# zzuiekongning/MGDT-YOLO

Hardware: AMD Instinct MI355X
Metric: images/sec @640x640 bs=32 per GPU, detection forward + NMS (whole job: 1 GPU(s)) (higher is better)
Workload: dtype bf16; 1 GPU; mspa_c2f_gd_yolov8-n (MSPA-C2f + GD neck + Detect, nc=80) 640x640 inference, batch 32/GPU: forward + decode + NMS(conf 0.25, iou 0.7), hipGraph replay, 4 batches in flight (one captured graph per resident batch, replayed round-robin on 4 streams); global_batch=32, parallelism=replicas x1 (batch-sharded, no data-path collective), rccl_ranks=1, input=bfloat16 NCHW images, 8 different batches resident in HBM (600 MiB) cycled, detections_last_step=9600, weights=seeded random init (no checkpoints offline), batches_in_flight=4

## Files before the change

### mgdt_yolo_amd/csrc/inject_fused.hip

```cpp
#include "conv_igemm_kernel.h"

struct InjArgs {
  const char* x; int xsn, xsh, xsw; uint32_t x_bytes;
  const char* ga; const char* gf; int gsn, gsh, gsw;
  char* y; int ysn, ysh, ysw; uint32_t y_bytes;
  const char* wpk; const float* bias;
  int N, H, W, Cin, Cout, Hg, Wg, PH, PW, tiles_x, tiles_y;
  FastDiv fd_tx, fd_ty;
  float ry, rx;
};

constexpr int INJ_TH = 4, INJ_TW = 16, INJ_THREADS = 256, INJ_CPAD = 8;

__device__ __host__ inline void inj_lerp_r(int o, float scale, int isz, int& i0, int& i1, float& l1) {
#pragma clang fp contract(off)
  float src = scale * ((float)o + 0.5f) - 0.5f;
  if (src < 0.f) src = 0.f;
  i0 = (int)src;
  if (i0 > isz - 1) i0 = isz - 1;
  i1 = i0 + (i0 < isz - 1 ? 1 : 0);
  l1 = src - (float)i0;
}
__device__ __host__ inline void inj_lerp(int o, int isz, int osz, int& i0, int& i1, float& l1) {
#pragma clang fp contract(off)
  inj_lerp_r(o, (float)isz / (float)osz, isz, i0, i1, l1);
}

typedef __attribute__((ext_vector_type(2))) float inj_f32x2;
typedef __attribute__((ext_vector_type(2))) __bf16 inj_bf16x2;
typedef __attribute__((ext_vector_type(4))) unsigned int u32x4;
__device__ __forceinline__ uint32_t inj_pk_bf16(float lo, float hi) {
  return __builtin_bit_cast(uint32_t, __builtin_convertvector(inj_f32x2{lo, hi}, inj_bf16x2));
}
__device__ __forceinline__ float inj_bf16_lo(uint32_t w) { return __uint_as_float(w << 16); }
__device__ __forceinline__ float inj_bf16_hi(uint32_t w) { return __uint_as_float(w & 0xffff0000u); }

struct InjGeo { int n, ty, tx, py0, px0, ph, pw; uint32_t pwm; };
__device__ __forceinline__ uint32_t inj_pw_magic(int pw) {
  uint32_t m = (uint32_t)(65536.f * __builtin_amdgcn_rcpf((float)pw));
  m -= (m * (uint32_t)pw > 65536u);
  m += ((m + 1) * (uint32_t)pw <= 65536u);
  return m + 1;
}
template <int TH>
__device__ __forceinline__ InjGeo inj_geom(const InjArgs& a, int patch) {
  InjGeo q;
  const uint32_t row = fdiv((uint32_t)patch, a.fd_tx);
  q.tx = patch - (int)row * a.tiles_x;
  q.n = (int)fdiv(row, a.fd_ty);
  q.ty = (int)row - q.n * a.tiles_y;
  int py1, px1, t0, t1; float tl;
  inj_lerp_r(q.ty * TH, a.ry, a.Hg, q.py0, t1, tl);
  inj_lerp_r(min(q.ty * TH + TH - 1, a.H - 1), a.ry, a.Hg, t0, py1, tl);
  inj_lerp_r(q.tx * INJ_TW, a.rx, a.Wg, q.px0, t1, tl);
  inj_lerp_r(min(q.tx * INJ_TW + INJ_TW - 1, a.W - 1), a.rx, a.Wg, t0, px1, tl);
  q.ph = py1 - q.py0 + 1; q.pw = px1 - q.px0 + 1;
  q.pwm = inj_pw_magic(q.pw);
  return q;
}

template <typename T, int KC, int NB>
__global__ __launch_bounds__(INJ_THREADS) void conv1x1_inject_kernel(const InjArgs a) {
  typedef typename Piece<T>::frag frag;
  constexpr int SZ = (int)sizeof(T);
  constexpr int CS = NB * 16 + INJ_CPAD;
  extern __shared__ __attribute__((aligned(16))) char smem[];
  char* wl = smem;
  T* sg = (T*)(smem + (size_t)KC * NB * 1024);
  T* sf = sg + (size_t)a.PH * a.PW * CS;
  const int tid = threadIdx.x, lane = tid & 63;
  const int wave = __builtin_amdgcn_readfirstlane(tid >> 6);
  const int r = lane & 15, g = lane >> 4;
  for (int i = tid; i < KC * NB * 64; i += INJ_THREADS) ((uint4*)wl)[i] = ((const uint4*)a.wpk)[i];
  const __amdgpu_buffer_rsrc_t xrs = __builtin_amdgcn_make_buffer_rsrc((void*)a.x, 0, a.x_bytes, 0x00020000);
  const __amdgpu_buffer_rsrc_t yrs = __builtin_amdgcn_make_buffer_rsrc((void*)a.y, 0, a.y_bytes, 0x00020000);
  const char* const wlane = wl + lane * 16;
  const int npatch = a.N * a.tiles_x * a.tiles_y;
#pragma unroll 1
  for (int patch = blockIdx.x; patch < npatch; patch += gridDim.x) {
  const InjGeo q = inj_geom<INJ_TH>(a, patch);
  const int n = q.n, ty = q.ty, tx = q.tx, py0 = q.py0, px0 = q.px0, ph = q.ph, pw = q.pw;
  const int oy = ty * INJ_TH + wave, ox = tx * INJ_TW + r;
  const bool pv = oy < a.H && ox < a.W;

  const int xo = pv ? n * a.xsn + oy * a.xsh + ox * a.xsw : MGDT_OOB;
  frag P[KC];
#pragma unroll
  for (int kc = 0; kc < KC; ++kc) {
    const int cb = (kc * 4 + g) * 16;
    P[kc] = __builtin_bit_cast(frag, __builtin_amdgcn_raw_buffer_load_b128(xrs, (cb < a.Cin * SZ) ? (uint32_t)(xo + cb) : (uint32_t)MGDT_OOB, 0, 0));
  }
  __syncthreads();
  {
    constexpr int VPP = NB * 16 / 8;
    const int nvec = ph * pw * VPP;
    for (int i = tid; i < nvec; i += INJ_THREADS) {
      const int v = i % VPP, p = i / VPP;
      const int sy = (int)(((uint32_t)p * q.pwm) >> 16), sx = p - sy * pw;
      const long go = (long)n * a.gsn + (long)(py0 + sy) * a.gsh + (long)(px0 + sx) * a.gsw + v * 16;
      const uint4 va = *(const uint4*)(a.ga + go), vf = *(const uint4*)(a.gf + go);
      *(uint4*)((char*)sg + ((size_t)p * CS + v * 8) * SZ) = va;
      *(uint4*)((char*)sf + ((size_t)p * CS + v * 8) * SZ) = vf;
    }
  }
  __syncthreads();

  f32x4 acc[NB];
#pragma unroll
  for (int nb = 0; nb < NB; ++nb) acc[nb] = *(const f32x4*)(a.bias + nb * 16 + 4 * g);
#pragma unroll
  for (int kc = 0; kc < KC; ++kc)
#pragma unroll
    for (int nb = 0; nb < NB; ++nb) acc[nb] = mma(*(const frag*)(wlane + (kc * NB + nb) * 1024), P[kc], acc[nb]);

  int y0, y1, x0, x1; float wy1, wx1;
  inj_lerp_r(min(oy, a.H - 1), a.ry, a.Hg, y0, y1, wy1);
  inj_lerp_r(min(ox, a.W - 1), a.rx, a.Wg, x0, x1, wx1);
  const int o00 = ((y0 - py0) * pw + (x0 - px0)) * CS + 4 * g, o01 = ((y0 - py0) * pw + (x1 - px0)) * CS + 4 * g;
  const int o10 = ((y1 - py0) * pw + (x0 - px0)) * CS + 4 * g, o11 = ((y1 - py0) * pw + (x1 - px0)) * CS + 4 * g;
  const int yo = pv ? n * a.ysn + oy * a.ysh + ox * a.ysw : MGDT_OOB;
  auto ld = [&](const T* base, int off) __attribute__((always_inline)) {
    const bf16x4 v = *(const bf16x4*)(base + off);
    return f32x4{(float)v[0], (float)v[1], (float)v[2], (float)v[3]};
  };
  auto hs = [](f32x4 v) __attribute__((always_inline)) {
    f32x4 o;
#pragma unroll
    for (int j = 0; j < 4; ++j) o[j] = fminf(fmaxf(fmaf(v[j], 1.f / 6.f, 0.5f), 0.f), 1.f);
    return o;
  };
#pragma unroll
  for (int nb = 0; nb < NB; ++nb) {
    const int c = nb * 16;
    const f32x4 sig = (hs(ld(sg, o00 + c)) * (1.f - wx1) + hs(ld(sg, o01 + c)) * wx1) * (1.f - wy1) +
                      (hs(ld(sg, o10 + c)) * (1.f - wx1) + hs(ld(sg, o11 + c)) * wx1) * wy1;
    const f32x4 feat = (ld(sf, o00 + c) * (1.f - wx1) + ld(sf, o01 + c) * wx1) * (1.f - wy1) +
                       (ld(sf, o10 + c) * (1.f - wx1) + ld(sf, o11 + c) * wx1) * wy1;
    f32x4 loc;
#pragma unroll
    for (int j = 0; j < 4; ++j) loc[j] = (float)(T)acc[nb][j];
    bstore4<T>(yrs, (uint32_t)yo + (uint32_t)((c + 4 * g) * SZ), loc * sig + feat);
  }
  }
}

struct InjConvArgs {
  InjArgs a;
  const char* gx; int gxsn, gxsh, gxsw; uint32_t gx_bytes;
  const char* wg; const float* bias_g;
  const char* w2; const float* bias2;
  char* y2; int y2sn, y2sh, y2sw; uint32_t y2_bytes;
  int C2, act2;
};

template <int KC, int NB, int NB2, int TH, bool GCONV>
__global__ __launch_bounds__(64 * TH) void conv1x1_inject_conv_kernel(const InjConvArgs A) {
  typedef bf16 T;
  typedef bf16x8 frag;
  const InjArgs& a = A.a;
  constexpr int SZ = 2, THREADS = 64 * TH;
  constexpr int CS = NB * 16 + INJ_CPAD;
  constexpr int KC2 = NB / 2;
  extern __shared__ __attribute__((aligned(16))) char smem[];
  char* wl = smem;
  char* w2l = smem + (size_t)KC * NB * 1024;
  T* sg = (T*)(w2l + (size_t)KC2 * NB2 * 1024);
  T* sf = sg + (size_t)a.PH * a.PW * CS;
  char* hgT = (char*)sg;
  char* gfT = hgT + (size_t)NB * 2 * 1024;

  const int tid = threadIdx.x, lane = tid & 63;
  const int wave = __builtin_amdgcn_readfirstlane(tid >> 6);
  const int r = lane & 15, g = lane >> 4;
  {
    constexpr int W1 = KC * NB * 64, W2 = KC2 * NB2 * 64, N1 = (W1 + THREADS - 1) / THREADS, N2 = (W2 + THREADS - 1) / THREADS;
    uint4 t1[N1], t2[N2];
#pragma unroll
    for (int u = 0; u < N1; ++u) t1[u] = ((const uint4*)a.wpk)[min(tid + u * THREADS, W1 - 1)];
#pragma unroll
    for (int u = 0; u < N2; ++u) t2[u] = ((const uint4*)A.w2)[min(tid + u * THREADS, W2 - 1)];
#pragma unroll
    for (int u = 0; u < N1; ++u) if (tid + u * THREADS < W1) ((uint4*)wl)[tid + u * THREADS] = t1[u];
#pragma unroll
    for (int u = 0; u < N2; ++u) if (tid + u * THREADS < W2) ((uint4*)w2l)[tid + u * THREADS] = t2[u];
  }
  if (GCONV) {
    for (int i = tid; i < NB * 2 * 2 * 64; i += THREADS) ((uint4*)hgT)[i] = make_uint4(0u, 0u, 0u, 0u);
  }
  const __amdgpu_buffer_rsrc_t xrs = __builtin_amdgcn_make_buffer_rsrc((void*)a.x, 0, a.x_bytes, 0x00020000);
  const __amdgpu_buffer_rsrc_t yrs = __builtin_amdgcn_make_buffer_rsrc((void*)A.y2, 0, A.y2_bytes, 0x00020000);
  const char* const wlane = wl + lane * 16;
  const char* const w2lane = w2l + lane * 16;
  static_assert(!GCONV || (2 * NB) % TH == 0, "cout blocks per wave");
  constexpr int GB = GCONV ? (2 * NB) / TH : 1;
  bf16x8 Ag[GB];
  if (GCONV) {
#pragma unroll
    for (int t = 0; t < GB; ++t) Ag[t] = *(const bf16x8*)(A.wg + ((size_t)(wave * GB + t) * 64 + lane) * 16);
  }
  const __amdgpu_buffer_rsrc_t grs = __builtin_amdgcn_make_buffer_rsrc((void*)(GCONV ? A.gx : a.x), 0, GCONV ? A.gx_bytes : 0u, 0x00020000);
  const int npatch = a.N * a.tiles_x * a.tiles_y;
  constexpr int NG = 4;
  f32x4 bgl[GB];
  if (GCONV) {
#pragma unroll
    for (int t = 0; t < GB; ++t) {
      const float b = A.bias_g[(wave * GB + t) * 16 + r];
      bgl[t] = f32x4{b, b, b, b};
    }
  }
  auto request = [&](int patch, InjGeo& gq, frag(&Pq)[KC], frag(&Bq)[NG]) __attribute__((always_inline)) {
    const bool live = patch < npatch;
    gq = inj_geom<TH>(a, live ? patch : 0);
    const int oy = gq.ty * TH + wave, ox = gq.tx * INJ_TW + r;
    const int xo = (live && oy < a.H && ox < a.W) ? gq.n * a.xsn + oy * a.xsh + ox * a.xsw : MGDT_OOB;
#pragma unroll
    for (int kc = 0; kc < KC; ++kc) {
      const int cb = (kc * 4 + g) * 16;
      Pq[kc] = __builtin_bit_cast(frag, __builtin_amdgcn_raw_buffer_load_b128(xrs, (cb < a.Cin * SZ) ? (uint32_t)(xo + cb) : (uint32_t)MGDT_OOB, 0, 0));
    }
    if (GCONV) {
      const int npx = gq.ph * gq.pw;
      const int gbase = gq.n * A.gxsn + gq.py0 * A.gxsh + gq.px0 * A.gxsw + g * 16;
#pragma unroll
      for (int grp = 0; grp < NG; ++grp) {
        const int p = grp * 16 + r;
        const int sy = (int)(((uint32_t)p * gq.pwm) >> 16), sx = p - sy * gq.pw;
        const uint32_t go = (live && p < npx) ? (uint32_t)(gbase + sy * A.gxsh + sx * A.gxsw) : (uint32_t)MGDT_OOB;
        Bq[grp] = __builtin_bit_cast(frag, __builtin_amdgcn_raw_buffer_load_b128(grs, go, 0, 0));
      }
    }
  };
  frag P[KC], Pn[KC], Bgc[NG], Bgn[NG];
  InjGeo q, qn;
  request((int)blockIdx.x, q, P, Bgc);
#pragma unroll 1
  for (int patch = blockIdx.x; patch < npatch; patch += gridDim.x) {
    const int n = q.n, py0 = q.py0, px0 = q.px0, ph = q.ph, pw = q.pw;
    const int oy = q.ty * TH + wave, ox = q.tx * INJ_TW + r;
    const bool pv = oy < a.H && ox < a.W;
    __syncthreads();
    if (GCONV) {
      const int npx = ph * pw;
#pragma unroll
      for (int grp = 0; grp < NG; ++grp) {
        if (grp * 16 >= npx) break;
        const frag Bg = Bgc[grp];
#pragma unroll
        for (int t = 0; t < GB; ++t) {
          const int nbg = wave * GB + t;
          const f32x4 o = mma(Bg, Ag[t], bgl[t]);
          const bool gate = nbg < NB;
          uint2 w = make_uint2(inj_pk_bf16(o[0], o[1]), inj_pk_bf16(o[2], o[3]));
          if (gate) {
            auto hsig = [](float v) __attribute__((always_inline)) { return fminf(fmaxf(fmaf(v, 1.f / 6.f, 0.5f), 0.f), 1.f); };
            w = make_uint2(inj_pk_bf16(hsig(inj_bf16_lo(w.x)), hsig(inj_bf16_hi(w.x))), inj_pk_bf16(hsig(inj_bf16_lo(w.y)), hsig(inj_bf16_hi(w.y))));
          }
          *(uint2*)((gate ? hgT : gfT) + ((size_t)((nbg % NB) * 2 + (grp >> 1)) * 64 + ((grp & 1) * 2 + (g >> 1)) * 16 + r) * 16 + 8 * (g & 1)) = w;
        }
      }
    } else {
      constexpr int VPP = NB * 16 / 8;
      const int nvec = ph * pw * VPP;
      for (int i = tid; i < nvec; i += THREADS) {
        const int v = i % VPP, p = i / VPP;
        const int sy = (int)(((uint32_t)p * q.pwm) >> 16), sx = p - sy * pw;
        const long go = (long)n * a.gsn + (long)(py0 + sy) * a.gsh + (long)(px0 + sx) * a.gsw + v * 16;
        const uint4 va = *(const uint4*)(a.ga + go), vf = *(const uint4*)(a.gf + go);
        *(uint4*)((char*)sg + ((size_t)p * CS + v * 8) * SZ) = va;
        *(uint4*)((char*)sf + ((size_t)p * CS + v * 8) * SZ) = vf;
      }
    }
    request(patch + (int)gridDim.x, qn, Pn, Bgn);
    f32x4 acc[NB];
#pragma unroll
    for (int nb = 0; nb < NB; ++nb) acc[nb] = *(const f32x4*)(a.bias + nb * 16 + 4 * g);
#pragma unroll
    for (int kc = 0; kc < KC; ++kc)
#pragma unroll
      for (int nb = 0; nb < NB; ++nb) acc[nb] = mma(*(const frag*)(wlane + (kc * NB + nb) * 1024), P[kc], acc[nb]);
    int y0, y1, x0, x1; float wy1, wx1;
    inj_lerp_r(min(oy, a.H - 1), a.ry, a.Hg, y0, y1, wy1);
    inj_lerp_r(min(ox, a.W - 1), a.rx, a.Wg, x0, x1, wx1);
    frag WB[2];
    if (GCONV) {
      const int dy = (y1 - y0) * pw, dx = x1 - x0;
      const int s00 = (y0 - py0) * pw + (x0 - px0) - 8 * g;
      const float w00 = (1.f - wy1) * (1.f - wx1), w01 = (1.f - wy1) * wx1, w10 = wy1 * (1.f - wx1), w11 = wy1 * wx1;
      float m0, m1, m2, m3;
      {
#pragma clang fp contract(off)
        if (dx == 0 && dy == 0) { m0 = w00 + w01 + w10 + w11; m1 = m2 = m3 = 0.f; }
        else if (dx == 0) { m0 = w00 + w01; m2 = w10 + w11; m1 = m3 = 0.f; }
        else if (dy == 0) { m0 = w00 + w10; m1 = w01 + w11; m2 = m3 = 0.f; }
        else { m0 = w00; m1 = w01; m2 = w10; m3 = w11; }
      }
      const int sl[4] = {s00, dx ? s00 + dx : -2, dy ? s00 + dy : -2, (dx && dy) ? s00 + dy + dx : -2};
      const float mw[4] = {m0, m1, m2, m3};
      int wd[4]; uint32_t bits[4];
#pragma unroll
      for (int t = 0; t < 4; ++t) {
        wd[t] = sl[t] >> 1;
        bits[t] = (uint32_t)__builtin_bit_cast(unsigned short, (bf16)mw[t]) << ((sl[t] & 1) * 16);
      }
#pragma unroll
      for (int kc = 0; kc < 2; ++kc) {
        u32x4 wv;
#pragma unroll
        for (int k = 0; k < 4; ++k)
          wv[k] = (wd[0] == kc * 16 + k ? bits[0] : 0u) | (wd[1] == kc * 16 + k ? bits[1] : 0u) | (wd[2] == kc * 16 + k ? bits[2] : 0u) |
                  (wd[3] == kc * 16 + k ? bits[3] : 0u);
        WB[kc] = __builtin_bit_cast(frag, wv);
      }
    }
    __syncthreads();
    const int o00 = ((y0 - py0) * pw + (x0 - px0)) * CS + 4 * g, o01 = ((y0 - py0) * pw + (x1 - px0)) * CS + 4 * g;
    const int o10 = ((y1 - py0) * pw + (x0 - px0)) * CS + 4 * g, o11 = ((y1 - py0) * pw + (x1 - px0)) * CS + 4 * g;
    auto ld = [&](const T* base, int off) __attribute__((always_inline)) {
      const bf16x4 v = *(const bf16x4*)(base + off);
      return f32x4{(float)v[0], (float)v[1], (float)v[2], (float)v[3]};
    };
    auto hs = [](f32x4 v) __attribute__((always_inline)) {
      f32x4 o;
#pragma unroll
      for (int j = 0; j < 4; ++j) o[j] = fminf(fmaxf(fmaf(v[j], 1.f / 6.f, 0.5f), 0.f), 1.f);
      return o;
    };
    f32x4 acc2[NB2];
#pragma unroll
    for (int nb = 0; nb < NB2; ++nb) acc2[nb] = *(const f32x4*)(A.bias2 + nb * 16 + 4 * g);
    const char* const hglane = hgT + lane * 16;
    const char* const gflane = gfT + lane * 16;
#pragma unroll
    for (int j = 0; j < KC2; ++j) {
      u32x4 B2w;
#pragma unroll
      for (int h = 0; h < 2; ++h) {
        const int nb = 2 * j + h;
        f32x4 sig, feat;
        if constexpr (GCONV) {
          sig = f32x4{0.f, 0.f, 0.f, 0.f}; feat = f32x4{0.f, 0.f, 0.f, 0.f};
#pragma unroll
          for (int kc = 0; kc < 2; ++kc) {
            sig = mma(*(const frag*)(hglane + (nb * 2 + kc) * 1024), WB[kc], sig);
            feat = mma(*(const frag*)(gflane + (nb * 2 + kc) * 1024), WB[kc], feat);
          }
        } else {
          const int c = nb * 16;
          sig = (hs(ld(sg, o00 + c)) * (1.f - wx1) + hs(ld(sg, o01 + c)) * wx1) * (1.f - wy1) +
                (hs(ld(sg, o10 + c)) * (1.f - wx1) + hs(ld(sg, o11 + c)) * wx1) * wy1;
          feat = (ld(sf, o00 + c) * (1.f - wx1) + ld(sf, o01 + c) * wx1) * (1.f - wy1) +
                 (ld(sf, o10 + c) * (1.f - wx1) + ld(sf, o11 + c) * wx1) * wy1;
        }
        const uint32_t a01 = inj_pk_bf16(acc[nb][0], acc[nb][1]), a23 = inj_pk_bf16(acc[nb][2], acc[nb][3]);
        B2w[h * 2] = inj_pk_bf16(inj_bf16_lo(a01) * sig[0] + feat[0], inj_bf16_hi(a01) * sig[1] + feat[1]);
        B2w[h * 2 + 1] = inj_pk_bf16(inj_bf16_lo(a23) * sig[2] + feat[2], inj_bf16_hi(a23) * sig[3] + feat[3]);
      }
      const frag B2 = __builtin_bit_cast(frag, B2w);
#pragma unroll
      for (int nb = 0; nb < NB2; ++nb) acc2[nb] = mma(*(const frag*)(w2lane + (j * NB2 + nb) * 1024), B2, acc2[nb]);
    }
    const int yo = pv ? n * A.y2sn + oy * A.y2sh + ox * A.y2sw : MGDT_OOB;
#pragma unroll
    for (int nb = 0; nb < NB2; ++nb) {
      const int c = nb * 16 + 4 * g;
      f32x4 v = acc2[nb];
#pragma unroll
      for (int i = 0; i < 4; ++i) v[i] = A.act2 == MGDT_ACT_SILU ? v[i] * fast_sigmoid(v[i]) : act_apply(v[i], A.act2);
      bstore4<T>(yrs, c < A.C2 ? (uint32_t)yo + (uint32_t)(c * SZ) : (uint32_t)MGDT_OOB, v);
    }
#pragma unroll
    for (int kc = 0; kc < KC; ++kc) P[kc] = Pn[kc];
#pragma unroll
    for (int grp = 0; grp < NG; ++grp) Bgc[grp] = Bgn[grp];
    q = qn;
  }
}

static int inj_kc(int cin) { return (cin + 31) / 32; }

static void inj_patch(int H, int W, int Hg, int Wg, int* PH, int* PW) {
  int ph = 1, pw = 1, a0, a1, b0, b1; float t;
  for (int ty = 0; ty * INJ_TH < H; ++ty) {
    inj_lerp(ty * INJ_TH, Hg, H, a0, a1, t);
    inj_lerp(std::min(ty * INJ_TH + INJ_TH - 1, H - 1), Hg, H, b0, b1, t);
    ph = std::max(ph, b1 - a0 + 1);
  }
  for (int tx = 0; tx * INJ_TW < W; ++tx) {
    inj_lerp(tx * INJ_TW, Wg, W, a0, a1, t);
    inj_lerp(std::min(tx * INJ_TW + INJ_TW - 1, W - 1), Wg, W, b0, b1, t);
    pw = std::max(pw, b1 - a0 + 1);
  }
  *PH = ph; *PW = pw;
}

static size_t inj_lds(int kc, int nb, int PH, int PW) { return (size_t)kc * nb * 1024 + (size_t)2 * PH * PW * (nb * 16 + INJ_CPAD) * 2; }

extern "C" int mgdt_conv1x1_inject_supported(int cin, int cout, int h, int w, int hg, int wg, int dtype) {
  if (dtype != MGDT_BF16 || cin % 8 || cin > 128 || (cout != 128 && cout != 256) || h < hg || w < wg || hg < 1 || wg < 1) return 0;
  int PH, PW;
  inj_patch(h, w, hg, wg, &PH, &PW);
  return inj_lds(inj_kc(cin), cout / 16, PH, PW) <= 80 * 1024;
}

template <int KC, int NB>
static int inj_launch(const InjArgs& a, size_t lds, hipStream_t st) {
  if (int rc = lds_optin<conv1x1_inject_kernel<bf16, KC, NB>>("conv1x1_inject", 80 * 1024)) return rc;
  conv1x1_inject_kernel<bf16, KC, NB><<<std::min(a.N * a.tiles_x * a.tiles_y, 512), INJ_THREADS, lds, st>>>(a);
  MGDT_CHECK_LAUNCH("conv1x1_inject_fwd");
  return MGDT_OK;
}

extern "C" int mgdt_conv1x1_inject_fwd(const mgdt_view* x, const void* packed_w, const float* bias, const mgdt_view* ga, const mgdt_view* gf,
                                       const mgdt_view* y, int dtype, mgdt_stream s) {
  if (!view_ok(x) || !view_ok(ga) || !view_ok(gf) || !view_ok(y) || !packed_w || !bias) MGDT_FAIL(MGDT_BAD_ARG, "conv1x1_inject: null/empty argument");
  if (!mgdt_conv1x1_inject_supported(x->c, y->c, y->h, y->w, ga->h, ga->w, dtype))
    MGDT_FAIL(MGDT_BAD_SHAPE, "conv1x1_inject: shapes/dtype not covered (see mgdt_conv1x1_inject_supported)");
  const int sz = 2;
  if (x->n != y->n || x->h != y->h || x->w != y->w || ga->n != y->n || gf->n != y->n || ga->c != y->c || gf->c != y->c || ga->h != gf->h || ga->w != gf->w ||
      ga->sn != gf->sn || ga->sh != gf->sh || ga->sw != gf->sw)
    MGDT_FAIL(MGDT_BAD_SHAPE, "conv1x1_inject: x/y spatial sizes, ga/gf shapes and layouts must match");
  InjArgs a;
  memset(&a, 0, sizeof(a));
  const char* yp = nullptr;
  auto nhwc8 = [&](const mgdt_view* v) { return v->sc == 1 && view_aligned(v, 8, sz); };
  if (!nhwc8(ga) || !nhwc8(gf) || !bind_view(x, sz, {8, true, 0, 0, false}, &a.x, &a.xsn, &a.xsh, &a.xsw, &a.x_bytes) ||
      !bind_view(y, sz, {4, true, 0, 0, false}, &yp, &a.ysn, &a.ysh, &a.ysw, &a.y_bytes))
    MGDT_FAIL(MGDT_BAD_SHAPE, "conv1x1_inject: views must be aligned NHWC (sc == 1) and < 2 GiB");
  a.y = (char*)yp;
  a.ga = (const char*)ga->p; a.gf = (const char*)gf->p; a.gsn = (int)(ga->sn * sz); a.gsh = (int)(ga->sh * sz); a.gsw = (int)(ga->sw * sz);
  a.wpk = (const char*)packed_w; a.bias = bias;
  a.N = y->n; a.H = y->h; a.W = y->w; a.Cin = x->c; a.Cout = y->c; a.Hg = ga->h; a.Wg = ga->w;
  inj_patch(a.H, a.W, a.Hg, a.Wg, &a.PH, &a.PW);
  a.tiles_x = cdiv(a.W, INJ_TW); a.tiles_y = cdiv(a.H, INJ_TH);
  a.fd_tx = make_fastdiv((uint32_t)a.tiles_x); a.fd_ty = make_fastdiv((uint32_t)a.tiles_y);
  a.ry = (float)a.Hg / (float)a.H; a.rx = (float)a.Wg / (float)a.W;
  const int kc = inj_kc(a.Cin), nb = a.Cout / 16;
  const size_t lds = inj_lds(kc, nb, a.PH, a.PW);
  hipStream_t st = (hipStream_t)s;
#define INJ_CASE(K, B) if (kc == K && nb == B) return inj_launch<K, B>(a, lds, st);
  INJ_CASE(1, 8) INJ_CASE(2, 8) INJ_CASE(3, 8) INJ_CASE(4, 8) INJ_CASE(1, 16) INJ_CASE(2, 16) INJ_CASE(3, 16) INJ_CASE(4, 16)
#undef INJ_CASE
  MGDT_FAIL(MGDT_BAD_SHAPE, "conv1x1_inject: no kernel for kc=%d nb=%d", kc, nb);
}

constexpr int INJ2_TH = 8;
static void inj_patch_th(int H, int W, int Hg, int Wg, int TH, int* PH, int* PW) {
  int ph = 1, pw = 1, a0, a1, b0, b1; float t;
  for (int ty = 0; ty * TH < H; ++ty) {
    inj_lerp(ty * TH, Hg, H, a0, a1, t);
    inj_lerp(std::min(ty * TH + TH - 1, H - 1), Hg, H, b0, b1, t);
    ph = std::max(ph, b1 - a0 + 1);
  }
  for (int tx = 0; tx * INJ_TW < W; ++tx) {
    inj_lerp(tx * INJ_TW, Wg, W, a0, a1, t);
    inj_lerp(std::min(tx * INJ_TW + INJ_TW - 1, W - 1), Wg, W, b0, b1, t);
    pw = std::max(pw, b1 - a0 + 1);
  }
  *PH = ph; *PW = pw;
}
static size_t inj2_lds(int kc, int nb, int nb2, int PH, int PW) {
  return (size_t)kc * nb * 1024 + (size_t)(nb / 2) * nb2 * 1024 + std::max((size_t)2 * PH * PW * (nb * 16 + INJ_CPAD) * 2, (size_t)2 * nb * 2 * 1024);
}

extern "C" int mgdt_conv1x1_inject_conv_supported(int cin, int cmid, int cout2, int h, int w, int hg, int wg, int dtype) {
  if (dtype != MGDT_BF16 || cin % 8 || cin > 128 || cmid != 256 || cout2 % 16 || cout2 < 16 || cout2 > 64 || h < hg || w < wg || hg < 1 || wg < 1) return 0;
  int PH, PW;
  inj_patch_th(h, w, hg, wg, INJ2_TH, &PH, &PW);
  return PH * PW <= 64 && inj2_lds(inj_kc(cin), cmid / 16, cout2 / 16, PH, PW) <= 156 * 1024;
}

template <int KC, int NB2, bool GCONV>
static int inj2_launch(const InjConvArgs& A, size_t lds, hipStream_t st) {
  if (int rc = lds_optin<conv1x1_inject_conv_kernel<KC, 16, NB2, INJ2_TH, GCONV>>("conv1x1_inject_conv")) return rc;
  conv1x1_inject_conv_kernel<KC, 16, NB2, INJ2_TH, GCONV><<<std::min(A.a.N * A.a.tiles_x * A.a.tiles_y, 256), 64 * INJ2_TH, lds, st>>>(A);
  MGDT_CHECK_LAUNCH("conv1x1_inject_conv_fwd");
  return MGDT_OK;
}

extern "C" int mgdt_conv1x1_inject_conv_fwd(const mgdt_view* x, const void* packed_w, const float* bias, const mgdt_view* ga_in, const mgdt_view* gf_in,
                                            const mgdt_view* gsrc, const void* packed_wg, const float* bias_g, int cmid,
                                            const void* packed_w2, const float* bias2, int act2, const mgdt_view* y2, int dtype, mgdt_stream s) {
  const bool gconv = gsrc && gsrc->p;
  mgdt_view gav, gfv;
  if (gconv) {
    if (!view_ok(gsrc) || !packed_wg || !bias_g || gsrc->c != 32 || cmid != 256) MGDT_FAIL(MGDT_BAD_ARG, "conv1x1_inject_conv: global source must be a 32-channel view with its merged panel (cmid 256)");
    gav = *gsrc; gav.c = cmid; gfv = gav;
  } else {
    if (!view_ok(ga_in) || !view_ok(gf_in)) MGDT_FAIL(MGDT_BAD_ARG, "conv1x1_inject_conv: null/empty global maps");
    gav = *ga_in; gfv = *gf_in;
  }
  const mgdt_view* ga = &gav; const mgdt_view* gf = &gfv;
  if (!view_ok(x) || !view_ok(y2) || !packed_w || !bias || !packed_w2 || !bias2) MGDT_FAIL(MGDT_BAD_ARG, "conv1x1_inject_conv: null/empty argument");
  if (!mgdt_conv1x1_inject_conv_supported(x->c, ga->c, y2->c, x->h, x->w, ga->h, ga->w, dtype))
    MGDT_FAIL(MGDT_BAD_SHAPE, "conv1x1_inject_conv: shapes/dtype not covered (see mgdt_conv1x1_inject_conv_supported)");
  const int sz = 2;
  if (x->n != y2->n || x->h != y2->h || x->w != y2->w || ga->n != x->n || gf->n != x->n || gf->c != ga->c || ga->h != gf->h || ga->w != gf->w ||
      ga->sn != gf->sn || ga->sh != gf->sh || ga->sw != gf->sw)
    MGDT_FAIL(MGDT_BAD_SHAPE, "conv1x1_inject_conv: x/y2 spatial sizes, ga/gf shapes and layouts must match");
  InjConvArgs A;
  memset(&A, 0, sizeof(A));
  InjArgs& a = A.a;
  const ViewPolicy in16 = {8, true, 0, 0, false}, out8 = {4, true, 0, 0, false};
  const char* y2p = nullptr;
  auto nhwc8 = [&](const mgdt_view* v) { return v->sc == 1 && view_aligned(v, 8, sz); };
  if ((gconv ? !bind_view(gsrc, sz, in16, &A.gx, &A.gxsn, &A.gxsh, &A.gxsw, &A.gx_bytes) : !nhwc8(ga) || !nhwc8(gf)) ||
      !bind_view(x, sz, in16, &a.x, &a.xsn, &a.xsh, &a.xsw, &a.x_bytes) || !bind_view(y2, sz, out8, &y2p, &A.y2sn, &A.y2sh, &A.y2sw, &A.y2_bytes))
    MGDT_FAIL(MGDT_BAD_SHAPE, "conv1x1_inject_conv: views must be aligned NHWC (sc == 1) and < 2 GiB");
  A.y2 = (char*)y2p;
  if (gconv) { A.wg = (const char*)packed_wg; A.bias_g = bias_g; }
  a.ga = (const char*)ga->p; a.gf = (const char*)gf->p; a.gsn = (int)(ga->sn * sz); a.gsh = (int)(ga->sh * sz); a.gsw = (int)(ga->sw * sz);
  a.wpk = (const char*)packed_w; a.bias = bias;
  a.N = x->n; a.H = x->h; a.W = x->w; a.Cin = x->c; a.Cout = ga->c; a.Hg = ga->h; a.Wg = ga->w;
  inj_patch_th(a.H, a.W, a.Hg, a.Wg, INJ2_TH, &a.PH, &a.PW);
  a.tiles_x = cdiv(a.W, INJ_TW); a.tiles_y = cdiv(a.H, INJ2_TH);
  a.fd_tx = make_fastdiv((uint32_t)a.tiles_x); a.fd_ty = make_fastdiv((uint32_t)a.tiles_y);
  a.ry = (float)a.Hg / (float)a.H; a.rx = (float)a.Wg / (float)a.W;
  A.w2 = (const char*)packed_w2; A.bias2 = bias2; A.act2 = act2; A.C2 = y2->c;
  const int kc = inj_kc(a.Cin), nb2 = cdiv(y2->c, 16);
  const size_t lds = inj2_lds(kc, 16, nb2, a.PH, a.PW);
  hipStream_t st = (hipStream_t)s;
#define INJ2_CASE(K, B) if (kc == K && nb2 == B) return gconv ? inj2_launch<K, B, true>(A, lds, st) : inj2_launch<K, B, false>(A, lds, st);
  INJ2_CASE(1, 1) INJ2_CASE(1, 2) INJ2_CASE(1, 3) INJ2_CASE(1, 4) INJ2_CASE(2, 1) INJ2_CASE(2, 2) INJ2_CASE(2, 3) INJ2_CASE(2, 4)
  INJ2_CASE(3, 1) INJ2_CASE(3, 2) INJ2_CASE(3, 3) INJ2_CASE(3, 4) INJ2_CASE(4, 1) INJ2_CASE(4, 2) INJ2_CASE(4, 3) INJ2_CASE(4, 4)
#undef INJ2_CASE
  MGDT_FAIL(MGDT_BAD_SHAPE, "conv1x1_inject_conv: no kernel for kc=%d nb2=%d", kc, nb2);
}
```

Measured before the change: 43060 images/sec.

## Software-pipeline inject-conv GEMM fragments, skip unused WB chunks, add timing probe

In the fused inject+conv kernel, LDS weight fragments are now double-buffered around the first GEMM and the second-stage fragment loads, with sched barriers to force load/MFMA overlap. Bias loads are hoisted, and the gate/feature branch is specialised per wave at compile time. When a wave's bilinear-weight chunk is all zero, that chunk's MFMAs are skipped. An optional wall-clock instrumentation variant is added behind an env knob. The changes raise register pressure and add branchy specialisation.

Measured after the change: 43420 images/sec, median of 6. Within noise of the previous version (+0.8%).

```diff
diff --git a/mgdt_yolo_amd/csrc/inject_fused.hip b/mgdt_yolo_amd/csrc/inject_fused.hip
--- a/mgdt_yolo_amd/csrc/inject_fused.hip
+++ b/mgdt_yolo_amd/csrc/inject_fused.hip
@@ -151,9 +151,12 @@
   const char* w2; const float* bias2;
   char* y2; int y2sn, y2sh, y2sw; uint32_t y2_bytes;
   int C2, act2;
+  int noskip;
+  unsigned long long* dbg;
 };
-
-template <int KC, int NB, int NB2, int TH, bool GCONV>
+constexpr int INJ_DBG_WORDS = 10;
+
+template <int KC, int NB, int NB2, int TH, bool GCONV, bool DBG>
 __global__ __launch_bounds__(64 * TH) void conv1x1_inject_conv_kernel(const InjConvArgs A) {
   typedef bf16 T;
   typedef bf16x8 frag;
@@ -172,6 +175,16 @@
   const int tid = threadIdx.x, lane = tid & 63;
   const int wave = __builtin_amdgcn_readfirstlane(tid >> 6);
   const int r = lane & 15, g = lane >> 4;
+  const bool dbg = DBG && wave == 0;
+  uint32_t tk = 0, dsum = 0;
+  auto lap = [&](int k) __attribute__((always_inline)) {
+    if (dbg) { const uint32_t t = (uint32_t)wall_clock64(); dsum += lane == k ? t - tk : (k == 6 && lane == 7) ? 1u : 0u; tk = t; }
+  };
+  if (dbg) {
+    const unsigned long long t = wall_clock64();
+    tk = (uint32_t)t;
+    if (lane == 0) A.dbg[(size_t)blockIdx.x * INJ_DBG_WORDS] = t;
+  }
   {
     constexpr int W1 = KC * NB * 64, W2 = KC2 * NB2 * 64, N1 = (W1 + THREADS - 1) / THREADS, N2 = (W2 + THREADS - 1) / THREADS;
     uint4 t1[N1], t2[N2];
@@ -234,23 +247,43 @@
   frag P[KC], Pn[KC], Bgc[NG], Bgn[NG];
   InjGeo q, qn;
   request((int)blockIdx.x, q, P, Bgc);
+  lap(0);
 #pragma unroll 1
   for (int patch = blockIdx.x; patch < npatch; patch += gridDim.x) {
     const int n = q.n, py0 = q.py0, px0 = q.px0, ph = q.ph, pw = q.pw;
     const int oy = q.ty * TH + wave, ox = q.tx * INJ_TW + r;
     const bool pv = oy < a.H && ox < a.W;
+    constexpr bool ROOMY = KC <= 2;
+    f32x4 acc[NB], acc2[NB2];
+    auto biases = [&]() __attribute__((always_inline)) {
+#pragma unroll
+      for (int nb = 0; nb < NB; ++nb) acc[nb] = *(const f32x4*)(a.bias + nb * 16 + 4 * g);
+#pragma unroll
+      for (int nb = 0; nb < NB2; ++nb) acc2[nb] = *(const f32x4*)(A.bias2 + nb * 16 + 4 * g);
+      __builtin_amdgcn_sched_barrier(0);
+    };
+    if constexpr (ROOMY) biases();
     __syncthreads();
+    lap(1);
     if (GCONV) {
       const int npx = ph * pw;
+      static_assert(!GCONV || NB % GB == 0, "the blocks of a wave lie in one map");
+      auto build = [&](auto gate_c) __attribute__((always_inline)) {
+      constexpr bool gate = decltype(gate_c)::value;
 #pragma unroll
       for (int grp = 0; grp < NG; ++grp) {
         if (grp * 16 >= npx) break;
         const frag Bg = Bgc[grp];
+        constexpr int OG = ROOMY ? GB : 1;
+        f32x4 og[OG];
 #pragma unroll
         for (int t = 0; t < GB; ++t) {
+          if (t % OG == 0) {
+#pragma unroll
+            for (int u = 0; u < OG; ++u) og[u] = mma(Bg, Ag[t + u], bgl[t + u]);
+          }
           const int nbg = wave * GB + t;
-          const f32x4 o = mma(Bg, Ag[t], bgl[t]);
-          const bool gate = nbg < NB;
+          const f32x4 o = og[t % OG];
           uint2 w = make_uint2(inj_pk_bf16(o[0], o[1]), inj_pk_bf16(o[2], o[3]));
           if (gate) {
             auto hsig = [](float v) __attribute__((always_inline)) { return fminf(fmaxf(fmaf(v, 1.f / 6.f, 0.5f), 0.f), 1.f); };
@@ -259,6 +292,8 @@
           *(uint2*)((gate ? hgT : gfT) + ((size_t)((nbg % NB) * 2 + (grp >> 1)) * 64 + ((grp & 1) * 2 + (g >> 1)) * 16 + r) * 16 + 8 * (g & 1)) = w;
         }
       }
+      };
+      if (wave * GB < NB) build(std::true_type{}); else build(std::false_type{});
     } else {
       constexpr int VPP = NB * 16 / 8;
       const int nvec = ph * pw * VPP;
@@ -271,18 +306,35 @@
         *(uint4*)((char*)sf + ((size_t)p * CS + v * 8) * SZ) = vf;
       }
     }
+    lap(2);
+    if constexpr (!ROOMY) biases();
     request(patch + (int)gridDim.x, qn, Pn, Bgn);
-    f32x4 acc[NB];
-#pragma unroll
-    for (int nb = 0; nb < NB; ++nb) acc[nb] = *(const f32x4*)(a.bias + nb * 16 + 4 * g);
-#pragma unroll
-    for (int kc = 0; kc < KC; ++kc)
-#pragma unroll
-      for (int nb = 0; nb < NB; ++nb) acc[nb] = mma(*(const frag*)(wlane + (kc * NB + nb) * 1024), P[kc], acc[nb]);
+    {
+      constexpr int FB = ROOMY ? 4 : 2, NBATCH = KC * NB / FB;
+      static_assert(NB % FB == 0, "a batch stays inside one K chunk");
+      frag wf[2][FB];
+#pragma unroll
+      for (int i = 0; i < FB; ++i) wf[0][i] = *(const frag*)(wlane + i * 1024);
+#pragma unroll
+      for (int b = 0; b < NBATCH; ++b) {
+        if (b + 1 < NBATCH) {
+#pragma unroll
+          for (int i = 0; i < FB; ++i) wf[(b + 1) & 1][i] = *(const frag*)(wlane + ((b + 1) * FB + i) * 1024);
+        }
+        __builtin_amdgcn_sched_barrier(0);
+#pragma unroll
+        for (int i = 0; i < FB; ++i) {
+          const int kc = (b * FB + i) / NB, nb = (b * FB + i) % NB;
+          acc[nb] = mma(wf[b & 1][i], P[kc], acc[nb]);
+        }
+        __builtin_amdgcn_sched_barrier(0);
+      }
+    }
     int y0, y1, x0, x1; float wy1, wx1;
     inj_lerp_r(min(oy, a.H - 1), a.ry, a.Hg, y0, y1, wy1);
     inj_lerp_r(min(ox, a.W - 1), a.rx, a.Wg, x0, x1, wx1);
     frag WB[2];
+    bool used[2] = {true, true};
     if (GCONV) {
       const int dy = (y1 - y0) * pw, dx = x1 - x0;
       const int s00 = (y0 - py0) * pw + (x0 - px0) - 8 * g;
@@ -311,9 +363,12 @@
           wv[k] = (wd[0] == kc * 16 + k ? bits[0] : 0u) | (wd[1] == kc * 16 + k ? bits[1] : 0u) | (wd[2] == kc * 16 + k ? bits[2] : 0u) |
                   (wd[3] == kc * 16 + k ? bits[3] : 0u);
         WB[kc] = __builtin_bit_cast(frag, wv);
-      }
-    }
+        used[kc] = __builtin_amdgcn_ballot_w64((wv[0] | wv[1] | wv[2] | wv[3]) != 0u) != 0;
+      }
+    }
+    lap(3);
     __syncthreads();
+    lap(4);
     const int o00 = ((y0 - py0) * pw + (x0 - px0)) * CS + 4 * g, o01 = ((y0 - py0) * pw + (x1 - px0)) * CS + 4 * g;
     const int o10 = ((y1 - py0) * pw + (x0 - px0)) * CS + 4 * g, o11 = ((y1 - py0) * pw + (x1 - px0)) * CS + 4 * g;
     auto ld = [&](const T* base, int off) __attribute__((always_inline)) {
@@ -326,54 +381,93 @@
       for (int j = 0; j < 4; ++j) o[j] = fminf(fmaxf(fmaf(v[j], 1.f / 6.f, 0.5f), 0.f), 1.f);
       return o;
     };
-    f32x4 acc2[NB2];
-#pragma unroll
-    for (int nb = 0; nb < NB2; ++nb) acc2[nb] = *(const f32x4*)(A.bias2 + nb * 16 + 4 * g);
     const char* const hglane = hgT + lane * 16;
     const char* const gflane = gfT + lane * 16;
-#pragma unroll
-    for (int j = 0; j < KC2; ++j) {
-      u32x4 B2w;
-#pragma unroll
-      for (int h = 0; h < 2; ++h) {
-        const int nb = 2 * j + h;
-        f32x4 sig, feat;
+    const bool both = !GCONV || A.noskip || (used[0] && used[1]);
+    const int kf = (!both && !used[0]) ? 1 : 0;
+    auto tail = [&](auto both_c) __attribute__((always_inline)) {
+      constexpr bool BOTH = decltype(both_c)::value;
+      const char* const hg0 = BOTH ? hglane : hglane + kf * 1024;
+      const char* const gf0 = BOTH ? gflane : gflane + kf * 1024;
+      const frag WB0 = (BOTH || kf == 0) ? WB[0] : WB[1];
+      frag fr[2][4], w2f[NB2];
+      auto frags = [&](int nb, frag(&f)[4]) __attribute__((always_inline)) {
         if constexpr (GCONV) {
-          sig = f32x4{0.f, 0.f, 0.f, 0.f}; feat = f32x4{0.f, 0.f, 0.f, 0.f};
-#pragma unroll
-          for (int kc = 0; kc < 2; ++kc) {
-            sig = mma(*(const frag*)(hglane + (nb * 2 + kc) * 1024), WB[kc], sig);
-            feat = mma(*(const frag*)(gflane + (nb * 2 + kc) * 1024), WB[kc], feat);
+          f[0] = *(const frag*)(hg0 + nb * 2048); f[1] = *(const frag*)(gf0 + nb * 2048);
+          if constexpr (BOTH) { f[2] = *(const frag*)(hglane + nb * 2048 + 1024); f[3] = *(const frag*)(gflane + nb * 2048 + 1024); }
+        }
+      };
+      frags(0, fr[0]);
+#pragma unroll
+      for (int j = 0; j < KC2; ++j) {
+        u32x4 B2w;
+        if constexpr (ROOMY) {
+#pragma unroll
+          for (int nb = 0; nb < NB2; ++nb) w2f[nb] = *(const frag*)(w2lane + (j * NB2 + nb) * 1024);
+        }
+#pragma unroll
+        for (int h = 0; h < 2; ++h) {
+          const int nb = 2 * j + h;
+          f32x4 sig, feat;
+          if constexpr (GCONV) {
+            if (nb + 1 < NB) frags(nb + 1, fr[(nb + 1) & 1]);
+            __builtin_amdgcn_sched_barrier(0);
+            sig = mma(fr[nb & 1][0], WB0, f32x4{0.f, 0.f, 0.f, 0.f});
+            feat = mma(fr[nb & 1][1], WB0, f32x4{0.f, 0.f, 0.f, 0.f});
+            if constexpr (BOTH) {
+              sig = mma(fr[nb & 1][2], WB[1], sig);
+              feat = mma(fr[nb & 1][3], WB[1], feat);
+            }
+          } else {
+            const int c = nb * 16;
+            sig = (hs(ld(sg, o00 + c)) * (1.f - wx1) + hs(ld(sg, o01 + c)) * wx1) * (1.f - wy1) +
+                  (hs(ld(sg, o10 + c)) * (1.f - wx1) + hs(ld(sg, o11 + c)) * wx1) * wy1;
+            feat = (ld(sf, o00 + c) * (1.f - wx1) + ld(sf, o01 + c) * wx1) * (1.f - wy1) +
+                   (ld(sf, o10 + c) * (1.f - wx1) + ld(sf, o11 + c) * wx1) * wy1;
           }
-        } else {
-          const int c = nb * 16;
-          sig = (hs(ld(sg, o00 + c)) * (1.f - wx1) + hs(ld(sg, o01 + c)) * wx1) * (1.f - wy1) +
-                (hs(ld(sg, o10 + c)) * (1.f - wx1) + hs(ld(sg, o11 + c)) * wx1) * wy1;
-          feat = (ld(sf, o00 + c) * (1.f - wx1) + ld(sf, o01 + c) * wx1) * (1.f - wy1) +
-                 (ld(sf, o10 + c) * (1.f - wx1) + ld(sf, o11 + c) * wx1) * wy1;
+          const uint32_t a01 = inj_pk_bf16(acc[nb][0], acc[nb][1]), a23 = inj_pk_bf16(acc[nb][2], acc[nb][3]);
+          B2w[h * 2] = inj_pk_bf16(inj_bf16_lo(a01) * sig[0] + feat[0], inj_bf16_hi(a01) * sig[1] + feat[1]);
+          B2w[h * 2 + 1] = inj_pk_bf16(inj_bf16_lo(a23) * sig[2] + feat[2], inj_bf16_hi(a23) * sig[3] + feat[3]);
         }
-        const uint32_t a01 = inj_pk_bf16(acc[nb][0], acc[nb][1]), a23 = inj_pk_bf16(acc[nb][2], acc[nb][3]);
-        B2w[h * 2] = inj_pk_bf16(inj_bf16_lo(a01) * sig[0] + feat[0], inj_bf16_hi(a01) * sig[1] + feat[1]);
-        B2w[h * 2 + 1] = inj_pk_bf16(inj_bf16_lo(a23) * sig[2] + feat[2], inj_bf16_hi(a23) * sig[3] + feat[3]);
-      }
-      const frag B2 = __builtin_bit_cast(frag, B2w);
-#pragma unroll
-      for (int nb = 0; nb < NB2; ++nb) acc2[nb] = mma(*(const frag*)(w2lane + (j * NB2 + nb) * 1024), B2, acc2[nb]);
-    }
+        const frag B2 = __builtin_bit_cast(frag, B2w);
+        if constexpr (!ROOMY) {
+#pragma unroll
+          for (int nb = 0; nb < NB2; ++nb) w2f[nb] = *(const frag*)(w2lane + (j * NB2 + nb) * 1024);
+        }
+#pragma unroll
+        for (int nb = 0; nb < NB2; ++nb) acc2[nb] = mma(w2f[nb], B2, acc2[nb]);
+      }
+    };
+    if (both) tail(std::true_type{}); else if constexpr (GCONV) tail(std::false_type{});
+    lap(5);
     const int yo = pv ? n * A.y2sn + oy * A.y2sh + ox * A.y2sw : MGDT_OOB;
+    if (A.act2 == MGDT_ACT_SILU) {
+#pragma unroll
+      for (int nb = 0; nb < NB2; ++nb)
+#pragma unroll
+        for (int i = 0; i < 4; ++i) acc2[nb][i] = acc2[nb][i] * fast_sigmoid(acc2[nb][i]);
+    } else {
+#pragma unroll
+      for (int nb = 0; nb < NB2; ++nb)
+#pragma unroll
+        for (int i = 0; i < 4; ++i) acc2[nb][i] = act_apply(acc2[nb][i], A.act2);
+    }
 #pragma unroll
     for (int nb = 0; nb < NB2; ++nb) {
       const int c = nb * 16 + 4 * g;
-      f32x4 v = acc2[nb];
-#pragma unroll
-      for (int i = 0; i < 4; ++i) v[i] = A.act2 == MGDT_ACT_SILU ? v[i] * fast_sigmoid(v[i]) : act_apply(v[i], A.act2);
-      bstore4<T>(yrs, c < A.C2 ? (uint32_t)yo + (uint32_t)(c * SZ) : (uint32_t)MGDT_OOB, v);
+      bstore4<T>(yrs, c < A.C2 ? (uint32_t)yo + (uint32_t)(c * SZ) : (uint32_t)MGDT_OOB, acc2[nb]);
     }
 #pragma unroll
     for (int kc = 0; kc < KC; ++kc) P[kc] = Pn[kc];
 #pragma unroll
     for (int grp = 0; grp < NG; ++grp) Bgc[grp] = Bgn[grp];
     q = qn;
+    lap(6);
+  }
+  if (dbg) {
+    unsigned long long* const w = A.dbg + (size_t)blockIdx.x * INJ_DBG_WORDS;
+    if (lane < 8) w[1 + lane] = dsum;
+    if (lane == 0) w[9] = wall_clock64();
   }
 }
 
@@ -472,9 +566,35 @@
 
 template <int KC, int NB2, bool GCONV>
 static int inj2_launch(const InjConvArgs& A, size_t lds, hipStream_t st) {
-  if (int rc = lds_optin<conv1x1_inject_conv_kernel<KC, 16, NB2, INJ2_TH, GCONV>>("conv1x1_inject_conv")) return rc;
-  conv1x1_inject_conv_kernel<KC, 16, NB2, INJ2_TH, GCONV><<<std::min(A.a.N * A.a.tiles_x * A.a.tiles_y, 256), 64 * INJ2_TH, lds, st>>>(A);
+  if (int rc = lds_optin<conv1x1_inject_conv_kernel<KC, 16, NB2, INJ2_TH, GCONV, false>>("conv1x1_inject_conv")) return rc;
+  if constexpr (GCONV) {
+    if (int rc = lds_optin<conv1x1_inject_conv_kernel<KC, 16, NB2, INJ2_TH, true, true>>("conv1x1_inject_conv")) return rc;
+  }
+  static StampBuf stamps;
+  const int grid = std::min(A.a.N * A.a.tiles_x * A.a.tiles_y, 256);
+  InjConvArgs B = A;
+  const bool dbg = GCONV && knob_set("MGDT_INJ_DBG");
+  if (dbg && !stamps.ensure((size_t)grid * INJ_DBG_WORDS)) MGDT_FAIL(MGDT_WORKSPACE, "conv1x1_inject_conv: no memory for the MGDT_INJ_DBG stamps");
+  B.dbg = dbg ? stamps.p : nullptr;
+  B.noskip = knob_unless0("MGDT_INJ_SKIP") ? 0 : 1;
+  if (dbg) conv1x1_inject_conv_kernel<KC, 16, NB2, INJ2_TH, true, GCONV><<<grid, 64 * INJ2_TH, lds, st>>>(B);
+  else conv1x1_inject_conv_kernel<KC, 16, NB2, INJ2_TH, GCONV, false><<<grid, 64 * INJ2_TH, lds, st>>>(B);
   MGDT_CHECK_LAUNCH("conv1x1_inject_conv_fwd");
+  if (dbg) {
+    const std::vector<unsigned long long> h = stamps.read((size_t)grid * INJ_DBG_WORDS, st);
+    unsigned long long t0 = ~0ull, t9 = 0; double sum[8] = {0, 0, 0, 0, 0, 0, 0, 0}, life = 0, life_long = 0;
+    unsigned long long most = 0; int n_long = 0;
+    for (int i = 0; i < grid; ++i) most = std::max(most, h[(size_t)i * INJ_DBG_WORDS + 8]);
+    for (int i = 0; i < grid; ++i) {
+      const unsigned long long* w = &h[(size_t)i * INJ_DBG_WORDS];
+      t0 = std::min(t0, w[0]); t9 = std::max(t9, w[9]); life += (double)(w[9] - w[0]);
+      if (w[8] == most) { life_long += (double)(w[9] - w[0]); ++n_long; }
+      for (int j = 0; j < 8; ++j) sum[j] += (double)w[1 + j];
+    }
+    fprintf(stderr, "conv1x1_inject_conv<%d,%d,%s,%s> x10ns: %d WGs, %zu B LDS, span %llu; %d WGs with %llu patches live %.0f; avg per WG: life %.0f = panels+first request %.0f + over %.2f patches: "
+            "barrier1 %.0f build %.0f request+gemm+taps %.0f barrier2 %.0f bilinear+cv1 %.0f epilogue+stores %.0f\n", KC, NB2, GCONV ? "gconv" : "maps", B.noskip ? "both chunks for every wave (MGDT_INJ_SKIP=0)" : "one-chunk waves skip", grid, lds,
+            t9 - t0, n_long, most, life_long / n_long, life / grid, sum[0] / grid, sum[7] / grid, sum[1] / grid, sum[2] / grid, sum[3] / grid, sum[4] / grid, sum[5] / grid, sum[6] / grid);
+  }
   return MGDT_OK;
 }
 
```
